# Xiuyu-Li/q-diffusion

Hardware: NVIDIA H100
Metric: images_per_sec (higher is better)
Workload: dtype int8 (W4/W8 codes x A8 codes, int32 accumulate; fp32 norms/softmax)

## Files before the change

q-diffusion_b200/csrc/attention_wg.cuh:

```cuda
#pragma once
#include "attention.cuh"
#include "ptx.cuh"

namespace qd {

__device__ __forceinline__ void wgmma_ra_s8s8_n64(uint32_t* d, const uint32_t (&a)[4], uint64_t db, uint32_t scale_d) {
  asm volatile(
      "{\n\t.reg .pred p;\n\t"
      "setp.ne.b32 p, %37, 0;\n\t"
      "wgmma.mma_async.sync.aligned.m64n64k32.s32.s8.s8 "
      "{%0, %1, %2, %3, %4, %5, %6, %7, %8, %9, %10, %11, %12, %13, %14, %15, %16, %17, %18, %19, %20, %21, %22, %23, %24, %25, %26, %27, %28, %29, %30, %31}, {%32, %33, %34, %35}, %36, p;\n\t}\n"
      : "+r"(d[0]), "+r"(d[1]), "+r"(d[2]), "+r"(d[3]), "+r"(d[4]), "+r"(d[5]), "+r"(d[6]), "+r"(d[7]), "+r"(d[8]), "+r"(d[9]), "+r"(d[10]), "+r"(d[11]), "+r"(d[12]), "+r"(d[13]), "+r"(d[14]), "+r"(d[15]), "+r"(d[16]), "+r"(d[17]), "+r"(d[18]), "+r"(d[19]), "+r"(d[20]), "+r"(d[21]), "+r"(d[22]), "+r"(d[23]), "+r"(d[24]), "+r"(d[25]), "+r"(d[26]), "+r"(d[27]), "+r"(d[28]), "+r"(d[29]), "+r"(d[30]), "+r"(d[31])
      : "r"(a[0]), "r"(a[1]), "r"(a[2]), "r"(a[3]), "l"(db), "r"(scale_d));
}
__device__ __forceinline__ void wgmma_ra_u8u8_n64(uint32_t* d, const uint32_t (&a)[4], uint64_t db, uint32_t scale_d) {
  asm volatile(
      "{\n\t.reg .pred p;\n\t"
      "setp.ne.b32 p, %37, 0;\n\t"
      "wgmma.mma_async.sync.aligned.m64n64k32.s32.u8.u8 "
      "{%0, %1, %2, %3, %4, %5, %6, %7, %8, %9, %10, %11, %12, %13, %14, %15, %16, %17, %18, %19, %20, %21, %22, %23, %24, %25, %26, %27, %28, %29, %30, %31}, {%32, %33, %34, %35}, %36, p;\n\t}\n"
      : "+r"(d[0]), "+r"(d[1]), "+r"(d[2]), "+r"(d[3]), "+r"(d[4]), "+r"(d[5]), "+r"(d[6]), "+r"(d[7]), "+r"(d[8]), "+r"(d[9]), "+r"(d[10]), "+r"(d[11]), "+r"(d[12]), "+r"(d[13]), "+r"(d[14]), "+r"(d[15]), "+r"(d[16]), "+r"(d[17]), "+r"(d[18]), "+r"(d[19]), "+r"(d[20]), "+r"(d[21]), "+r"(d[22]), "+r"(d[23]), "+r"(d[24]), "+r"(d[25]), "+r"(d[26]), "+r"(d[27]), "+r"(d[28]), "+r"(d[29]), "+r"(d[30]), "+r"(d[31])
      : "r"(a[0]), "r"(a[1]), "r"(a[2]), "r"(a[3]), "l"(db), "r"(scale_d));
}
__device__ __forceinline__ void wgmma_ra_f16_n64(float* d, const uint32_t (&a)[4], uint64_t db, uint32_t scale_d) {
  asm volatile(
      "{\n\t.reg .pred p;\n\t"
      "setp.ne.b32 p, %37, 0;\n\t"
      "wgmma.mma_async.sync.aligned.m64n64k16.f32.f16.f16 "
      "{%0, %1, %2, %3, %4, %5, %6, %7, %8, %9, %10, %11, %12, %13, %14, %15, %16, %17, %18, %19, %20, %21, %22, %23, %24, %25, %26, %27, %28, %29, %30, %31}, {%32, %33, %34, %35}, %36, p, 1, 1, 0;\n\t}\n"
      : "+f"(d[0]), "+f"(d[1]), "+f"(d[2]), "+f"(d[3]), "+f"(d[4]), "+f"(d[5]), "+f"(d[6]), "+f"(d[7]), "+f"(d[8]), "+f"(d[9]), "+f"(d[10]), "+f"(d[11]), "+f"(d[12]), "+f"(d[13]), "+f"(d[14]), "+f"(d[15]), "+f"(d[16]), "+f"(d[17]), "+f"(d[18]), "+f"(d[19]), "+f"(d[20]), "+f"(d[21]), "+f"(d[22]), "+f"(d[23]), "+f"(d[24]), "+f"(d[25]), "+f"(d[26]), "+f"(d[27]), "+f"(d[28]), "+f"(d[29]), "+f"(d[30]), "+f"(d[31])
      : "r"(a[0]), "r"(a[1]), "r"(a[2]), "r"(a[3]), "l"(db), "r"(scale_d));
}
__device__ __forceinline__ void wgmma_ra_u8u8_n24(uint32_t* d, const uint32_t (&a)[4], uint64_t db, uint32_t scale_d) {
  asm volatile(
      "{\n\t.reg .pred p;\n\t"
      "setp.ne.b32 p, %17, 0;\n\t"
      "wgmma.mma_async.sync.aligned.m64n24k32.s32.u8.u8 "
      "{%0, %1, %2, %3, %4, %5, %6, %7, %8, %9, %10, %11}, {%12, %13, %14, %15}, %16, p;\n\t}\n"
      : "+r"(d[0]), "+r"(d[1]), "+r"(d[2]), "+r"(d[3]), "+r"(d[4]), "+r"(d[5]), "+r"(d[6]), "+r"(d[7]), "+r"(d[8]), "+r"(d[9]), "+r"(d[10]), "+r"(d[11])
      : "r"(a[0]), "r"(a[1]), "r"(a[2]), "r"(a[3]), "l"(db), "r"(scale_d));
}
__device__ __forceinline__ void wgmma_ra_u8s8_n24(uint32_t* d, const uint32_t (&a)[4], uint64_t db, uint32_t scale_d) {
  asm volatile(
      "{\n\t.reg .pred p;\n\t"
      "setp.ne.b32 p, %17, 0;\n\t"
      "wgmma.mma_async.sync.aligned.m64n24k32.s32.u8.s8 "
      "{%0, %1, %2, %3, %4, %5, %6, %7, %8, %9, %10, %11}, {%12, %13, %14, %15}, %16, p;\n\t}\n"
      : "+r"(d[0]), "+r"(d[1]), "+r"(d[2]), "+r"(d[3]), "+r"(d[4]), "+r"(d[5]), "+r"(d[6]), "+r"(d[7]), "+r"(d[8]), "+r"(d[9]), "+r"(d[10]), "+r"(d[11])
      : "r"(a[0]), "r"(a[1]), "r"(a[2]), "r"(a[3]), "l"(db), "r"(scale_d));
}
__device__ __forceinline__ void wgmma_ra_u8u8_n32(uint32_t* d, const uint32_t (&a)[4], uint64_t db, uint32_t scale_d) {
  asm volatile(
      "{\n\t.reg .pred p;\n\t"
      "setp.ne.b32 p, %21, 0;\n\t"
      "wgmma.mma_async.sync.aligned.m64n32k32.s32.u8.u8 "
      "{%0, %1, %2, %3, %4, %5, %6, %7, %8, %9, %10, %11, %12, %13, %14, %15}, {%16, %17, %18, %19}, %20, p;\n\t}\n"
      : "+r"(d[0]), "+r"(d[1]), "+r"(d[2]), "+r"(d[3]), "+r"(d[4]), "+r"(d[5]), "+r"(d[6]), "+r"(d[7]), "+r"(d[8]), "+r"(d[9]), "+r"(d[10]), "+r"(d[11]), "+r"(d[12]), "+r"(d[13]), "+r"(d[14]), "+r"(d[15])
      : "r"(a[0]), "r"(a[1]), "r"(a[2]), "r"(a[3]), "l"(db), "r"(scale_d));
}
__device__ __forceinline__ void wgmma_ra_u8s8_n32(uint32_t* d, const uint32_t (&a)[4], uint64_t db, uint32_t scale_d) {
  asm volatile(
      "{\n\t.reg .pred p;\n\t"
      "setp.ne.b32 p, %21, 0;\n\t"
      "wgmma.mma_async.sync.aligned.m64n32k32.s32.u8.s8 "
      "{%0, %1, %2, %3, %4, %5, %6, %7, %8, %9, %10, %11, %12, %13, %14, %15}, {%16, %17, %18, %19}, %20, p;\n\t}\n"
      : "+r"(d[0]), "+r"(d[1]), "+r"(d[2]), "+r"(d[3]), "+r"(d[4]), "+r"(d[5]), "+r"(d[6]), "+r"(d[7]), "+r"(d[8]), "+r"(d[9]), "+r"(d[10]), "+r"(d[11]), "+r"(d[12]), "+r"(d[13]), "+r"(d[14]), "+r"(d[15])
      : "r"(a[0]), "r"(a[1]), "r"(a[2]), "r"(a[3]), "l"(db), "r"(scale_d));
}
__device__ __forceinline__ void wgmma_ra_u8u8_n48(uint32_t* d, const uint32_t (&a)[4], uint64_t db, uint32_t scale_d) {
  asm volatile(
      "{\n\t.reg .pred p;\n\t"
      "setp.ne.b32 p, %29, 0;\n\t"
      "wgmma.mma_async.sync.aligned.m64n48k32.s32.u8.u8 "
      "{%0, %1, %2, %3, %4, %5, %6, %7, %8, %9, %10, %11, %12, %13, %14, %15, %16, %17, %18, %19, %20, %21, %22, %23}, {%24, %25, %26, %27}, %28, p;\n\t}\n"
      : "+r"(d[0]), "+r"(d[1]), "+r"(d[2]), "+r"(d[3]), "+r"(d[4]), "+r"(d[5]), "+r"(d[6]), "+r"(d[7]), "+r"(d[8]), "+r"(d[9]), "+r"(d[10]), "+r"(d[11]), "+r"(d[12]), "+r"(d[13]), "+r"(d[14]), "+r"(d[15]), "+r"(d[16]), "+r"(d[17]), "+r"(d[18]), "+r"(d[19]), "+r"(d[20]), "+r"(d[21]), "+r"(d[22]), "+r"(d[23])
      : "r"(a[0]), "r"(a[1]), "r"(a[2]), "r"(a[3]), "l"(db), "r"(scale_d));
}
__device__ __forceinline__ void wgmma_ra_u8s8_n48(uint32_t* d, const uint32_t (&a)[4], uint64_t db, uint32_t scale_d) {
  asm volatile(
      "{\n\t.reg .pred p;\n\t"
      "setp.ne.b32 p, %29, 0;\n\t"
      "wgmma.mma_async.sync.aligned.m64n48k32.s32.u8.s8 "
      "{%0, %1, %2, %3, %4, %5, %6, %7, %8, %9, %10, %11, %12, %13, %14, %15, %16, %17, %18, %19, %20, %21, %22, %23}, {%24, %25, %26, %27}, %28, p;\n\t}\n"
      : "+r"(d[0]), "+r"(d[1]), "+r"(d[2]), "+r"(d[3]), "+r"(d[4]), "+r"(d[5]), "+r"(d[6]), "+r"(d[7]), "+r"(d[8]), "+r"(d[9]), "+r"(d[10]), "+r"(d[11]), "+r"(d[12]), "+r"(d[13]), "+r"(d[14]), "+r"(d[15]), "+r"(d[16]), "+r"(d[17]), "+r"(d[18]), "+r"(d[19]), "+r"(d[20]), "+r"(d[21]), "+r"(d[22]), "+r"(d[23])
      : "r"(a[0]), "r"(a[1]), "r"(a[2]), "r"(a[3]), "l"(db), "r"(scale_d));
}
__device__ __forceinline__ void wgmma_ra_u8s8_n64(uint32_t* d, const uint32_t (&a)[4], uint64_t db, uint32_t scale_d) {
  asm volatile(
      "{\n\t.reg .pred p;\n\t"
      "setp.ne.b32 p, %37, 0;\n\t"
      "wgmma.mma_async.sync.aligned.m64n64k32.s32.u8.s8 "
      "{%0, %1, %2, %3, %4, %5, %6, %7, %8, %9, %10, %11, %12, %13, %14, %15, %16, %17, %18, %19, %20, %21, %22, %23, %24, %25, %26, %27, %28, %29, %30, %31}, {%32, %33, %34, %35}, %36, p;\n\t}\n"
      : "+r"(d[0]), "+r"(d[1]), "+r"(d[2]), "+r"(d[3]), "+r"(d[4]), "+r"(d[5]), "+r"(d[6]), "+r"(d[7]), "+r"(d[8]), "+r"(d[9]), "+r"(d[10]), "+r"(d[11]), "+r"(d[12]), "+r"(d[13]), "+r"(d[14]), "+r"(d[15]), "+r"(d[16]), "+r"(d[17]), "+r"(d[18]), "+r"(d[19]), "+r"(d[20]), "+r"(d[21]), "+r"(d[22]), "+r"(d[23]), "+r"(d[24]), "+r"(d[25]), "+r"(d[26]), "+r"(d[27]), "+r"(d[28]), "+r"(d[29]), "+r"(d[30]), "+r"(d[31])
      : "r"(a[0]), "r"(a[1]), "r"(a[2]), "r"(a[3]), "l"(db), "r"(scale_d));
}
__device__ __forceinline__ void wgmma_ra_u8u8_n80(uint32_t* d, const uint32_t (&a)[4], uint64_t db, uint32_t scale_d) {
  asm volatile(
      "{\n\t.reg .pred p;\n\t"
      "setp.ne.b32 p, %45, 0;\n\t"
      "wgmma.mma_async.sync.aligned.m64n80k32.s32.u8.u8 "
      "{%0, %1, %2, %3, %4, %5, %6, %7, %8, %9, %10, %11, %12, %13, %14, %15, %16, %17, %18, %19, %20, %21, %22, %23, %24, %25, %26, %27, %28, %29, %30, %31, %32, %33, %34, %35, %36, %37, %38, %39}, {%40, %41, %42, %43}, %44, p;\n\t}\n"
      : "+r"(d[0]), "+r"(d[1]), "+r"(d[2]), "+r"(d[3]), "+r"(d[4]), "+r"(d[5]), "+r"(d[6]), "+r"(d[7]), "+r"(d[8]), "+r"(d[9]), "+r"(d[10]), "+r"(d[11]), "+r"(d[12]), "+r"(d[13]), "+r"(d[14]), "+r"(d[15]), "+r"(d[16]), "+r"(d[17]), "+r"(d[18]), "+r"(d[19]), "+r"(d[20]), "+r"(d[21]), "+r"(d[22]), "+r"(d[23]), "+r"(d[24]), "+r"(d[25]), "+r"(d[26]), "+r"(d[27]), "+r"(d[28]), "+r"(d[29]), "+r"(d[30]), "+r"(d[31]), "+r"(d[32]), "+r"(d[33]), "+r"(d[34]), "+r"(d[35]), "+r"(d[36]), "+r"(d[37]), "+r"(d[38]), "+r"(d[39])
      : "r"(a[0]), "r"(a[1]), "r"(a[2]), "r"(a[3]), "l"(db), "r"(scale_d));
}
__device__ __forceinline__ void wgmma_ra_u8s8_n80(uint32_t* d, const uint32_t (&a)[4], uint64_t db, uint32_t scale_d) {
  asm volatile(
      "{\n\t.reg .pred p;\n\t"
      "setp.ne.b32 p, %45, 0;\n\t"
      "wgmma.mma_async.sync.aligned.m64n80k32.s32.u8.s8 "
      "{%0, %1, %2, %3, %4, %5, %6, %7, %8, %9, %10, %11, %12, %13, %14, %15, %16, %17, %18, %19, %20, %21, %22, %23, %24, %25, %26, %27, %28, %29, %30, %31, %32, %33, %34, %35, %36, %37, %38, %39}, {%40, %41, %42, %43}, %44, p;\n\t}\n"
      : "+r"(d[0]), "+r"(d[1]), "+r"(d[2]), "+r"(d[3]), "+r"(d[4]), "+r"(d[5]), "+r"(d[6]), "+r"(d[7]), "+r"(d[8]), "+r"(d[9]), "+r"(d[10]), "+r"(d[11]), "+r"(d[12]), "+r"(d[13]), "+r"(d[14]), "+r"(d[15]), "+r"(d[16]), "+r"(d[17]), "+r"(d[18]), "+r"(d[19]), "+r"(d[20]), "+r"(d[21]), "+r"(d[22]), "+r"(d[23]), "+r"(d[24]), "+r"(d[25]), "+r"(d[26]), "+r"(d[27]), "+r"(d[28]), "+r"(d[29]), "+r"(d[30]), "+r"(d[31]), "+r"(d[32]), "+r"(d[33]), "+r"(d[34]), "+r"(d[35]), "+r"(d[36]), "+r"(d[37]), "+r"(d[38]), "+r"(d[39])
      : "r"(a[0]), "r"(a[1]), "r"(a[2]), "r"(a[3]), "l"(db), "r"(scale_d));
}
__device__ __forceinline__ void wgmma_ra_u8u8_n96(uint32_t* d, const uint32_t (&a)[4], uint64_t db, uint32_t scale_d) {
  asm volatile(
      "{\n\t.reg .pred p;\n\t"
      "setp.ne.b32 p, %53, 0;\n\t"
      "wgmma.mma_async.sync.aligned.m64n96k32.s32.u8.u8 "
      "{%0, %1, %2, %3, %4, %5, %6, %7, %8, %9, %10, %11, %12, %13, %14, %15, %16, %17, %18, %19, %20, %21, %22, %23, %24, %25, %26, %27, %28, %29, %30, %31, %32, %33, %34, %35, %36, %37, %38, %39, %40, %41, %42, %43, %44, %45, %46, %47}, {%48, %49, %50, %51}, %52, p;\n\t}\n"
      : "+r"(d[0]), "+r"(d[1]), "+r"(d[2]), "+r"(d[3]), "+r"(d[4]), "+r"(d[5]), "+r"(d[6]), "+r"(d[7]), "+r"(d[8]), "+r"(d[9]), "+r"(d[10]), "+r"(d[11]), "+r"(d[12]), "+r"(d[13]), "+r"(d[14]), "+r"(d[15]), "+r"(d[16]), "+r"(d[17]), "+r"(d[18]), "+r"(d[19]), "+r"(d[20]), "+r"(d[21]), "+r"(d[22]), "+r"(d[23]), "+r"(d[24]), "+r"(d[25]), "+r"(d[26]), "+r"(d[27]), "+r"(d[28]), "+r"(d[29]), "+r"(d[30]), "+r"(d[31]), "+r"(d[32]), "+r"(d[33]), "+r"(d[34]), "+r"(d[35]), "+r"(d[36]), "+r"(d[37]), "+r"(d[38]), "+r"(d[39]), "+r"(d[40]), "+r"(d[41]), "+r"(d[42]), "+r"(d[43]), "+r"(d[44]), "+r"(d[45]), "+r"(d[46]), "+r"(d[47])
      : "r"(a[0]), "r"(a[1]), "r"(a[2]), "r"(a[3]), "l"(db), "r"(scale_d));
}
__device__ __forceinline__ void wgmma_ra_u8s8_n96(uint32_t* d, const uint32_t (&a)[4], uint64_t db, uint32_t scale_d) {
  asm volatile(
      "{\n\t.reg .pred p;\n\t"
      "setp.ne.b32 p, %53, 0;\n\t"
      "wgmma.mma_async.sync.aligned.m64n96k32.s32.u8.s8 "
      "{%0, %1, %2, %3, %4, %5, %6, %7, %8, %9, %10, %11, %12, %13, %14, %15, %16, %17, %18, %19, %20, %21, %22, %23, %24, %25, %26, %27, %28, %29, %30, %31, %32, %33, %34, %35, %36, %37, %38, %39, %40, %41, %42, %43, %44, %45, %46, %47}, {%48, %49, %50, %51}, %52, p;\n\t}\n"
      : "+r"(d[0]), "+r"(d[1]), "+r"(d[2]), "+r"(d[3]), "+r"(d[4]), "+r"(d[5]), "+r"(d[6]), "+r"(d[7]), "+r"(d[8]), "+r"(d[9]), "+r"(d[10]), "+r"(d[11]), "+r"(d[12]), "+r"(d[13]), "+r"(d[14]), "+r"(d[15]), "+r"(d[16]), "+r"(d[17]), "+r"(d[18]), "+r"(d[19]), "+r"(d[20]), "+r"(d[21]), "+r"(d[22]), "+r"(d[23]), "+r"(d[24]), "+r"(d[25]), "+r"(d[26]), "+r"(d[27]), "+r"(d[28]), "+r"(d[29]), "+r"(d[30]), "+r"(d[31]), "+r"(d[32]), "+r"(d[33]), "+r"(d[34]), "+r"(d[35]), "+r"(d[36]), "+r"(d[37]), "+r"(d[38]), "+r"(d[39]), "+r"(d[40]), "+r"(d[41]), "+r"(d[42]), "+r"(d[43]), "+r"(d[44]), "+r"(d[45]), "+r"(d[46]), "+r"(d[47])
      : "r"(a[0]), "r"(a[1]), "r"(a[2]), "r"(a[3]), "l"(db), "r"(scale_d));
}
__device__ __forceinline__ void wgmma_ra_u8u8_n112(uint32_t* d, const uint32_t (&a)[4], uint64_t db, uint32_t scale_d) {
  asm volatile(
      "{\n\t.reg .pred p;\n\t"
      "setp.ne.b32 p, %61, 0;\n\t"
      "wgmma.mma_async.sync.aligned.m64n112k32.s32.u8.u8 "
      "{%0, %1, %2, %3, %4, %5, %6, %7, %8, %9, %10, %11, %12, %13, %14, %15, %16, %17, %18, %19, %20, %21, %22, %23, %24, %25, %26, %27, %28, %29, %30, %31, %32, %33, %34, %35, %36, %37, %38, %39, %40, %41, %42, %43, %44, %45, %46, %47, %48, %49, %50, %51, %52, %53, %54, %55}, {%56, %57, %58, %59}, %60, p;\n\t}\n"
      : "+r"(d[0]), "+r"(d[1]), "+r"(d[2]), "+r"(d[3]), "+r"(d[4]), "+r"(d[5]), "+r"(d[6]), "+r"(d[7]), "+r"(d[8]), "+r"(d[9]), "+r"(d[10]), "+r"(d[11]), "+r"(d[12]), "+r"(d[13]), "+r"(d[14]), "+r"(d[15]), "+r"(d[16]), "+r"(d[17]), "+r"(d[18]), "+r"(d[19]), "+r"(d[20]), "+r"(d[21]), "+r"(d[22]), "+r"(d[23]), "+r"(d[24]), "+r"(d[25]), "+r"(d[26]), "+r"(d[27]), "+r"(d[28]), "+r"(d[29]), "+r"(d[30]), "+r"(d[31]), "+r"(d[32]), "+r"(d[33]), "+r"(d[34]), "+r"(d[35]), "+r"(d[36]), "+r"(d[37]), "+r"(d[38]), "+r"(d[39]), "+r"(d[40]), "+r"(d[41]), "+r"(d[42]), "+r"(d[43]), "+r"(d[44]), "+r"(d[45]), "+r"(d[46]), "+r"(d[47]), "+r"(d[48]), "+r"(d[49]), "+r"(d[50]), "+r"(d[51]), "+r"(d[52]), "+r"(d[53]), "+r"(d[54]), "+r"(d[55])
      : "r"(a[0]), "r"(a[1]), "r"(a[2]), "r"(a[3]), "l"(db), "r"(scale_d));
}
__device__ __forceinline__ void wgmma_ra_u8s8_n112(uint32_t* d, const uint32_t (&a)[4], uint64_t db, uint32_t scale_d) {
  asm volatile(
      "{\n\t.reg .pred p;\n\t"
      "setp.ne.b32 p, %61, 0;\n\t"
      "wgmma.mma_async.sync.aligned.m64n112k32.s32.u8.s8 "
      "{%0, %1, %2, %3, %4, %5, %6, %7, %8, %9, %10, %11, %12, %13, %14, %15, %16, %17, %18, %19, %20, %21, %22, %23, %24, %25, %26, %27, %28, %29, %30, %31, %32, %33, %34, %35, %36, %37, %38, %39, %40, %41, %42, %43, %44, %45, %46, %47, %48, %49, %50, %51, %52, %53, %54, %55}, {%56, %57, %58, %59}, %60, p;\n\t}\n"
      : "+r"(d[0]), "+r"(d[1]), "+r"(d[2]), "+r"(d[3]), "+r"(d[4]), "+r"(d[5]), "+r"(d[6]), "+r"(d[7]), "+r"(d[8]), "+r"(d[9]), "+r"(d[10]), "+r"(d[11]), "+r"(d[12]), "+r"(d[13]), "+r"(d[14]), "+r"(d[15]), "+r"(d[16]), "+r"(d[17]), "+r"(d[18]), "+r"(d[19]), "+r"(d[20]), "+r"(d[21]), "+r"(d[22]), "+r"(d[23]), "+r"(d[24]), "+r"(d[25]), "+r"(d[26]), "+r"(d[27]), "+r"(d[28]), "+r"(d[29]), "+r"(d[30]), "+r"(d[31]), "+r"(d[32]), "+r"(d[33]), "+r"(d[34]), "+r"(d[35]), "+r"(d[36]), "+r"(d[37]), "+r"(d[38]), "+r"(d[39]), "+r"(d[40]), "+r"(d[41]), "+r"(d[42]), "+r"(d[43]), "+r"(d[44]), "+r"(d[45]), "+r"(d[46]), "+r"(d[47]), "+r"(d[48]), "+r"(d[49]), "+r"(d[50]), "+r"(d[51]), "+r"(d[52]), "+r"(d[53]), "+r"(d[54]), "+r"(d[55])
      : "r"(a[0]), "r"(a[1]), "r"(a[2]), "r"(a[3]), "l"(db), "r"(scale_d));
}

constexpr int ATW_STAGES = 4;
constexpr int ATW_THREADS = ATT_WARPS * 32;
__host__ __device__ constexpr int atw_nv(int DV) {
  return DV + 8 <= 24 ? 24 : DV + 8 <= 32 ? 32 : DV + 8 <= 48 ? 48 : DV + 8 <= 64 ? 64 : DV + 8 <= 80 ? 80 : DV + 8 <= 96 ? 96 : 112;
}
struct AtwSmem {
  int k_bytes, v_bytes, z_off, bar_off, total;
};
__host__ __device__ inline AtwSmem atw_smem(int P, int NV) {
  AtwSmem l;
  l.k_bytes = (ATT_BN * P + 1023) / 1024 * 1024;
  l.v_bytes = (NV * ATT_BN + 1023) / 1024 * 1024;
  l.z_off = ATW_STAGES * (l.k_bytes + l.v_bytes);
  l.bar_off = l.z_off + ATW_STAGES * ATT_BN * 4;
  l.total = l.bar_off + ATW_STAGES * 8 + ATW_STAGES * 4 + 1024;
  return l;
}
__device__ __forceinline__ uint64_t atw_desc(uint32_t addr, int row_bytes) {
  const uint64_t layout = row_bytes == 128 ? 1 : row_bytes == 64 ? 2 : 3;
  uint64_t d = (uint64_t)((addr & 0x3FFFF) >> 4);
  d |= (uint64_t)1 << 16;
  d |= (uint64_t)((8 * row_bytes) >> 4) << 32;
  d |= layout << 62;
  return d;
}

template <int N, bool VS>
__device__ __forceinline__ void atw_pv(uint32_t* d, const uint32_t (&a)[4], uint64_t db, uint32_t scale_d) {
  if constexpr (VS) {
    if constexpr (N == 24) wgmma_ra_u8s8_n24(d, a, db, scale_d);
    else if constexpr (N == 32) wgmma_ra_u8s8_n32(d, a, db, scale_d);
    else if constexpr (N == 48) wgmma_ra_u8s8_n48(d, a, db, scale_d);
    else if constexpr (N == 64) wgmma_ra_u8s8_n64(d, a, db, scale_d);
    else if constexpr (N == 80) wgmma_ra_u8s8_n80(d, a, db, scale_d);
    else if constexpr (N == 96) wgmma_ra_u8s8_n96(d, a, db, scale_d);
    else wgmma_ra_u8s8_n112(d, a, db, scale_d);
  } else {
    if constexpr (N == 24) wgmma_ra_u8u8_n24(d, a, db, scale_d);
    else if constexpr (N == 32) wgmma_ra_u8u8_n32(d, a, db, scale_d);
    else if constexpr (N == 48) wgmma_ra_u8u8_n48(d, a, db, scale_d);
    else if constexpr (N == 64) wgmma_ra_u8u8_n64(d, a, db, scale_d);
    else if constexpr (N == 80) wgmma_ra_u8u8_n80(d, a, db, scale_d);
    else if constexpr (N == 96) wgmma_ra_u8u8_n96(d, a, db, scale_d);
    else wgmma_ra_u8u8_n112(d, a, db, scale_d);
  }
}

template <int DQ, int DV, bool QK_SIGNED, bool V_SIGNED, bool SM16, bool F16, int MINB>
__global__ void __launch_bounds__(ATW_THREADS, MINB)
qattention_wg_kernel(const __grid_constant__ CUtensorMap tmK, const __grid_constant__ CUtensorMap tmV,
                     const qd_attention_desc p, int P) {
  constexpr int NV = atw_nv(DV);
  constexpr int NKC = DQ / 32;
  constexpr int NDT = DV / 8 + 1;
  constexpr int RB = F16 ? 2 * DV : DV;
  static_assert(!F16 || DV <= 64, "fp16 Q / K operands: d <= 64 keeps |S| below 2^22");
  static_assert(DV <= 96, "8-bit codes: the raw scores must stay below 2^23 (unsigned) / 2^22 (signed)");
  using SV = std::conditional_t<F16, float, uint32_t>;
  constexpr uint32_t MB = QK_SIGNED ? 0x4B400000u : 0x4B000000u;
  extern __shared__ uint8_t atw_raw[];
  uint8_t* smem = atw_raw + (((smem_u32(atw_raw) + 1023u) & ~1023u) - smem_u32(atw_raw));
  const AtwSmem lay = atw_smem(P, NV);
  uint64_t* full = reinterpret_cast<uint64_t*>(smem + lay.bar_off);
  int* released = reinterpret_cast<int*>(full + ATW_STAGES);

  const int warp = threadIdx.x >> 5, lane = threadIdx.x & 31;
  const int g = lane >> 2, t = lane & 3;
  const int bh = blockIdx.y;
  const int b = bh / p.heads, h = bh - b * p.heads;
  const int row0 = blockIdx.x * ATT_BM + warp * 16;
  const int ntiles = (p.Tk + ATT_BN - 1) / ATT_BN;
  const int nloads = 2 * ntiles;
  const bool has_zq = !F16 && p.zq != 0;
  const int* zrk_g = reinterpret_cast<const int*>(p.ws) + (long long)bh * (long long)att_ws_stride(p.Tk);

  for (int i = threadIdx.x; i < ATW_STAGES * (NV - DV) * ATT_BN; i += ATW_THREADS) {
    const int s = i / ((NV - DV) * ATT_BN), r = (i / ATT_BN) % (NV - DV) + DV, c = i % ATT_BN;
    smem[ATW_STAGES * lay.k_bytes + s * lay.v_bytes + r * ATT_BN + c] = r == DV ? 1 : 0;
  }
  if (threadIdx.x == 0) {
    tma_prefetch_desc(&tmK);
    tma_prefetch_desc(&tmV);
    for (int s = 0; s < ATW_STAGES; ++s) {
      mbar_init(&full[s], 1);
      released[s] = 0;
    }
    fence_mbar_init();
  }
  fence_proxy_async();
  __syncthreads();

  auto issue = [&](int L) {
    const int s = L % ATW_STAGES, pass = L / ntiles, tile = L - pass * ntiles;
    const int j0 = tile * ATT_BN;
    const uint32_t bytes = (uint32_t)(ATT_BN * P) + (pass ? (uint32_t)(ATT_BN * DV) : 0u) + (has_zq ? ATT_BN * 4u : 0u);
    mbar_arrive_expect_tx(&full[s], bytes);
    tma_load_2d(smem + s * lay.k_bytes, &tmK, &full[s], h * P, b * p.Tk + j0);
    if (pass) tma_load_2d(smem + ATW_STAGES * lay.k_bytes + s * lay.v_bytes, &tmV, &full[s], j0, bh * DV);
    if (has_zq) bulk_load_1d(smem + lay.z_off + s * ATT_BN * 4, zrk_g + j0, ATT_BN * 4, &full[s]);
  };
  if (threadIdx.x == 0)
    for (int L = 0; L < ATW_STAGES && L < nloads; ++L) issue(L);

  constexpr bool QRELOAD = DV == 48;
  uint32_t qf[NKC][4];
  const uint8_t* qbase = reinterpret_cast<const uint8_t*>(p.q) + (long long)b * p.Tq * p.ld_q + p.q_off + h * p.head_stride_q;
  const uint8_t* q0 = qbase + (long long)min(row0 + g, p.Tq - 1) * p.ld_q;
  const uint8_t* q1 = qbase + (long long)min(row0 + g + 8, p.Tq - 1) * p.ld_q;
  auto load_q = [&]() {
#pragma unroll
    for (int kc = 0; kc < NKC; ++kc) {
      const int c0 = kc * 32 + 4 * t, c1 = c0 + 16;
      qf[kc][0] = c0 < RB ? *reinterpret_cast<const uint32_t*>(q0 + c0) : 0u;
      qf[kc][1] = c0 < RB ? *reinterpret_cast<const uint32_t*>(q1 + c0) : 0u;
      qf[kc][2] = c1 < RB ? *reinterpret_cast<const uint32_t*>(q0 + c1) : 0u;
      qf[kc][3] = c1 < RB ? *reinterpret_cast<const uint32_t*>(q1 + c1) : 0u;
    }
  };
  if constexpr (!QRELOAD) load_q();
  const float c = p.sim_scale * 1.4426950408889634f;
  const bool ragged = (p.Tk % ATT_BN) != 0;
  float mi0 = -INFINITY, mi1 = -INFINITY;
  float l0 = 0.f, l1 = 0.f;

  auto issue_s = [&](SV (&s)[8][4], int L) {
    const int st = L % ATW_STAGES;
    if constexpr (QRELOAD) load_q();
    mbar_wait(&full[st], (uint32_t)(L / ATW_STAGES) & 1u);
    const uint64_t dK = atw_desc(smem_u32(smem + st * lay.k_bytes), P);
    wgmma_fence();
#pragma unroll
    for (int kc = 0; kc < NKC; ++kc) {
      if constexpr (F16) wgmma_ra_f16_n64(&s[0][0], qf[kc], dK + (uint64_t)(2 * kc), kc ? 1u : 0u);
      else if constexpr (QK_SIGNED) wgmma_ra_s8s8_n64(&s[0][0], qf[kc], dK + (uint64_t)(2 * kc), kc ? 1u : 0u);
      else wgmma_ra_u8u8_n64(&s[0][0], qf[kc], dK + (uint64_t)(2 * kc), kc ? 1u : 0u);
    }
    wgmma_commit();
  };
  auto scores = [&](SV (&s)[8][4], float (&f)[8][4], int L) {
    wgmma_fence_regs(reinterpret_cast<SV (&)[32]>(s));
    const int tile = L % ntiles, st = L % ATW_STAGES;
    if constexpr (F16) {
#pragma unroll
      for (int i = 0; i < 32; ++i) f[i >> 2][i & 3] = s[i >> 2][i & 3];
    } else {
      const uint32_t* sZrk = reinterpret_cast<const uint32_t*>(smem + lay.z_off + st * ATT_BN * 4);
#pragma unroll
      for (int nt = 0; nt < 8; ++nt) {
        float z0 = __uint_as_float(MB), z1 = z0;
        if (has_zq) {
          const uint2 z = *reinterpret_cast<const uint2*>(sZrk + 8 * nt + 2 * t);
          z0 = __uint_as_float(z.x + MB);
          z1 = __uint_as_float(z.y + MB);
        }
        f[nt][0] = __uint_as_float(s[nt][0] + MB) - z0; f[nt][1] = __uint_as_float(s[nt][1] + MB) - z1;
        f[nt][2] = __uint_as_float(s[nt][2] + MB) - z0; f[nt][3] = __uint_as_float(s[nt][3] + MB) - z1;
      }
    }
    if (ragged && tile == ntiles - 1) {
#pragma unroll
      for (int nt = 0; nt < 8; ++nt) {
        const int j = tile * ATT_BN + 8 * nt + 2 * t;
        if (j >= p.Tk) { f[nt][0] = -INFINITY; f[nt][2] = -INFINITY; }
        if (j + 1 >= p.Tk) { f[nt][1] = -INFINITY; f[nt][3] = -INFINITY; }
      }
    }
  };

  auto release = [&](int R) {
    __syncwarp();
    if (lane == 0) {
      const int s = R % ATW_STAGES;
      __threadfence_block();
      const int n = atomicAdd(&released[s], 1);
      if (n == ATT_WARPS * (R / ATW_STAGES + 1) - 1 && R + ATW_STAGES < nloads) {
        __threadfence_block();
        issue(R + ATW_STAGES);
      }
    }
  };

  for (int L = 0; L < ntiles; ++L) {
    SV sacc[8][4];
    issue_s(sacc, L);
    wgmma_wait<0>();
    float f[8][4];
    scores(sacc, f, L);
    release(L);
    float tm0 = f[0][0], tm1 = f[0][2];
#pragma unroll
    for (int nt = 0; nt < 8; ++nt) {
      tm0 = fmaxf(tm0, fmaxf(f[nt][0], f[nt][1]));
      tm1 = fmaxf(tm1, fmaxf(f[nt][2], f[nt][3]));
    }
    tm0 = fmaxf(tm0, __shfl_xor_sync(0xffffffffu, tm0, 1));
    tm0 = fmaxf(tm0, __shfl_xor_sync(0xffffffffu, tm0, 2));
    tm1 = fmaxf(tm1, __shfl_xor_sync(0xffffffffu, tm1, 1));
    tm1 = fmaxf(tm1, __shfl_xor_sync(0xffffffffu, tm1, 2));
    if (tm0 > mi0) { l0 *= (mi0 == -INFINITY) ? 0.f : ex2_approx((mi0 - tm0) * c); mi0 = tm0; }
    if (tm1 > mi1) { l1 *= (mi1 == -INFINITY) ? 0.f : ex2_approx((mi1 - tm1) * c); mi1 = tm1; }
    const float b0 = -mi0 * c, b1 = -mi1 * c;
    float a0 = 0.f, a1 = 0.f;
#pragma unroll
    for (int nt = 0; nt < 8; ++nt) {
      a0 += ex2_approx(fmaf(f[nt][0], c, b0)) + ex2_approx(fmaf(f[nt][1], c, b0));
      a1 += ex2_approx(fmaf(f[nt][2], c, b1)) + ex2_approx(fmaf(f[nt][3], c, b1));
    }
    l0 += a0;
    l1 += a1;
  }

  l0 += __shfl_xor_sync(0xffffffffu, l0, 1);
  l0 += __shfl_xor_sync(0xffffffffu, l0, 2);
  l1 += __shfl_xor_sync(0xffffffffu, l1, 1);
  l1 += __shfl_xor_sync(0xffffffffu, l1, 2);
  const float off0 = -mi0 * c + log2f(1.0f / (l0 * p.delta_w));
  const float off1 = -mi1 * c + log2f(1.0f / (l1 * p.delta_w));
  const float pmax = (float)p.p_qmax;
// ... 84 lines not shown
```

q-diffusion_b200/csrc/engine.cu:

```cuda
#include <cuda.h>
#include <cuda_runtime.h>
#include <cudaTypedefs.h>

#include <atomic>
#include <cstdarg>
#include <cstdio>
#include <cstdlib>
#include <cstring>
#include <mutex>
#include <new>
#include <utility>
#include <vector>

#include "../../include/qdiff_b200.h"
#include "attention.cuh"
#include "attention_wg.cuh"
#include "elem.cuh"
#include "gemm_i8.cuh"
#include "runtime.cuh"

namespace qdr {

thread_local char g_err[512] = "";
std::atomic<long long> g_launches{0};
// ... 664 lines not shown
bool im2col_vec(const qd_im2col_desc& d) {
  return (d.C % 16) == 0 && d.ld_dst == 9 * d.C && (d.ld_dst % 16) == 0 && aligned(d.src, 16) && aligned(d.dst, 16);
}

int validate_im2col(const qd_im2col_desc& d) {
  if (!d.src || !d.dst) return fail(QD_ERR_BAD_ARG, "im2col: null arg");
  if (d.B <= 0 || d.H <= 0 || d.W <= 0 || d.C <= 0 || d.Ho <= 0 || d.Wo <= 0 || d.stride <= 0)
    return fail(QD_ERR_BAD_ARG, "im2col: empty geometry");
  if (d.ld_dst < 9 * d.C) return fail(QD_ERR_BAD_ARG, "im2col: ld_dst too small");
  return QD_OK;
}

int launch_im2col(const qd_im2col_desc& d, cudaStream_t s) {
  if (int rc = validate_im2col(d)) return rc;
  if (im2col_vec(d)) {
    launch_k(qd::im2col_vec_kernel, grid_for((long long)d.B * d.Ho * d.Wo * 9 * (d.C / 16), 256), 256, 0, s, d);
    return check_launch("im2col_vec_kernel");
  }
  const long long total = (long long)d.B * d.Ho * d.Wo * d.ld_dst;
  launch_k(qd::im2col_kernel, grid_for(total, 256), 256, 0, s, d);
  return check_launch("im2col_kernel");
}

template <int DQ, int DV, bool QS, bool VS, bool S16, bool F16>
int launch_attention_inst(const qd_attention_desc& d, cudaStream_t s) {
  constexpr int MINB = (DV <= 48) ? 2 : 1;
  auto kern = qd::qattention_kernel<DQ, DV, QS, VS, S16, MINB, F16>;
  static std::atomic<unsigned long long> optin{0};
  if (int rc = ensure_smem_optin(kern, 200 * 1024, optin, "attention")) return rc;
  const bool zrk = !F16 && d.zq != 0;
  const qd::AttSmemLayout lay = qd::att_smem_layout(DQ, DV, d.Tk, zrk);
  if (lay.total > 200 * 1024) return fail(QD_ERR_UNSUPPORTED, "attention: Tk=%d needs %d B of shared memory", d.Tk, lay.total);
  if (zrk) {
    if (!d.ws) return fail(QD_ERR_BAD_ARG, "attention: workspace required when zq != 0");
    const int tk_pad = qd::att_ws_stride(d.Tk);
    launch_k(qd::att_krowsum_kernel<QS>, grid_for((long long)d.B * d.heads * tk_pad, 256), 256, 0, s, d, tk_pad, 0, 0);
    int rc = check_launch("att_krowsum_kernel");
    if (rc) return rc;
  }
  dim3 grid((d.Tq + qd::ATT_BM - 1) / qd::ATT_BM, d.B * d.heads);
  launch_k(kern, grid, qd::ATT_WARPS * 32, lay.total, s, d);
  return check_launch("qattention_kernel");
}

template <int DQ, int DV, bool F16 = false>
int launch_attention_t(const qd_attention_desc& d, cudaStream_t s) {
  const bool qs = d.q_signed != 0, vs = d.v_signed != 0, s16 = d.sm_bits > 8;
  if (qs && vs && s16) return launch_attention_inst<DQ, DV, true, true, true, F16>(d, s);
  if (qs && vs && !s16) return launch_attention_inst<DQ, DV, true, true, false, F16>(d, s);
  if (!qs && !vs && s16) return launch_attention_inst<DQ, DV, false, false, true, F16>(d, s);
  if (!qs && !vs && !s16) return launch_attention_inst<DQ, DV, false, false, false, F16>(d, s);
  return fail(QD_ERR_UNSUPPORTED, "attention: mixed signedness q=%d v=%d", d.q_signed, d.v_signed);
}

template <int DQ, int DV, bool QS, bool VS, bool S16>
int launch_attention_smallk_inst(const qd_attention_desc& d, cudaStream_t s) {
  constexpr int NKV = 3;
  auto kern = qd::qattention_smallk_kernel<DQ, DV, QS, VS, S16, NKV>;
  const int spw = d.Tq >= 2048 ? 4 : (d.Tq >= 512 ? 2 : 1);
  const int slabs = (d.Tq + 15) / 16;
  dim3 grid((slabs + spw * qd::ATS_WARPS - 1) / (spw * qd::ATS_WARPS), d.B * d.heads);
  launch_k(kern, grid, qd::ATS_WARPS * 32, qd::ats_smem_bytes<DQ, DV, NKV>(), s, d, spw);
  return check_launch("qattention_smallk_kernel");
}

template <int DQ, int DV>
int launch_attention_smallk(const qd_attention_desc& d, cudaStream_t s) {
  const bool qs = d.q_signed != 0, vs = d.v_signed != 0, s16 = d.sm_bits > 8;
  if (qs && vs && s16) return launch_attention_smallk_inst<DQ, DV, true, true, true>(d, s);
  if (qs && vs && !s16) return launch_attention_smallk_inst<DQ, DV, true, true, false>(d, s);
  if (!qs && !vs && s16) return launch_attention_smallk_inst<DQ, DV, false, false, true>(d, s);
  if (!qs && !vs && !s16) return launch_attention_smallk_inst<DQ, DV, false, false, false>(d, s);
  return fail(QD_ERR_UNSUPPORTED, "attention: mixed signedness q=%d v=%d", d.q_signed, d.v_signed);
}

bool attention_wg_eligible(const qd_attention_desc& d) {
  static const int forced_mma = [] { const char* e = getenv("QDIFF_ATTENTION"); return (e && !strcmp(e, "mma")) ? 1 : 0; }();
  if (forced_mma) return false;
  const int P = d.head_stride_q, rb = d.qk_f16 ? 2 * d.d : d.d;
  if (d.d != 16 && d.d != 24 && d.d != 32 && d.d != 40 && d.d != 48 && d.d != 64 && d.d != 80 && d.d != 96) return false;
  if (d.qk_f16 && d.d > 64) return false;
  if ((P != 32 && P != 64 && P != 128) || P < rb || d.head_stride_k != P) return false;
  if (d.q_off != 0 || d.k_off != 0 || (d.ld_k & 15) || (((uintptr_t)d.k) & 15) || (((uintptr_t)d.vt) & 15)) return false;
  if (d.v_off != 0 || d.head_stride_v != d.d || d.v_batch_stride != (long long)d.heads * d.d * d.ld_vt) return false;
  if (d.zq != 0 && !d.qk_f16 && !d.ws) return false;
  if (!d.qk_f16 && (d.zq > 255 || d.zq < (d.q_signed ? -255 : 0))) return false;
  return true;
}

template <int DQ, int DV, bool QS, bool VS, bool S16, bool F16>
int launch_attention_wg_inst(const qd_attention_desc& d, cudaStream_t s) {
  constexpr int MINB = DV <= 40 ? 2 : 1;
  auto kern = qd::qattention_wg_kernel<DQ, DV, QS, VS, S16, F16, MINB>;
  const int P = d.head_stride_q;
  const qd::AtwSmem lay = qd::atw_smem(P, qd::atw_nv(DV));
  static std::atomic<unsigned long long> optin{0};
  if (int rc = ensure_smem_optin(kern, 227 * 1024, optin, "attention_wg")) return rc;
  CUtensorMap tmK, tmV;
  {
    cuuint64_t dims[2] = {(cuuint64_t)d.ld_k, (cuuint64_t)d.B * d.Tk};
    cuuint64_t strides[1] = {(cuuint64_t)d.ld_k};
    cuuint32_t box[2] = {(cuuint32_t)P, (cuuint32_t)qd::ATT_BN};
    if (int rc = encode_u8_map(&tmK, d.k, 2, dims, strides, box, P)) return rc;
  }
  {
    cuuint64_t dims[2] = {(cuuint64_t)d.ld_vt, (cuuint64_t)d.B * d.heads * d.d};
    cuuint64_t strides[1] = {(cuuint64_t)d.ld_vt};
    cuuint32_t box[2] = {(cuuint32_t)qd::ATT_BN, (cuuint32_t)d.d};
    if (int rc = encode_u8_map(&tmV, d.vt, 2, dims, strides, box, 64)) return rc;
  }
  if (!F16 && d.zq != 0) {
    const int tk_pad = qd::att_ws_stride(d.Tk);
    launch_k(qd::att_krowsum_kernel<QS>, grid_for((long long)d.B * d.heads * tk_pad, 256), 256, 0, s, d, tk_pad, 0, 0);
    if (int rc = check_launch("att_krowsum_kernel")) return rc;
  }
  dim3 grid((d.Tq + qd::ATT_BM - 1) / qd::ATT_BM, d.B * d.heads);
  launch_k(kern, grid, qd::ATW_THREADS, lay.total, s, tmK, tmV, d, P);
  return check_launch("qattention_wg_kernel");
}

template <int DQ, int DV, bool F16>
int launch_attention_wg_t(const qd_attention_desc& d, cudaStream_t s) {
  const bool qs = d.q_signed != 0, vs = d.v_signed != 0, s16 = d.sm_bits > 8;
  if (qs && vs && s16) return launch_attention_wg_inst<DQ, DV, true, true, true, F16>(d, s);
  if (qs && vs && !s16) return launch_attention_wg_inst<DQ, DV, true, true, false, F16>(d, s);
  if (!qs && !vs && s16) return launch_attention_wg_inst<DQ, DV, false, false, true, F16>(d, s);
  if (!qs && !vs && !s16) return launch_attention_wg_inst<DQ, DV, false, false, false, F16>(d, s);
  return fail(QD_ERR_UNSUPPORTED, "attention: mixed signedness q=%d v=%d", d.q_signed, d.v_signed);
}

int launch_attention_wg(const qd_attention_desc& d, cudaStream_t s) {
  if (d.qk_f16) {
    switch (d.d) {
      case 16: return launch_attention_wg_t<32, 16, true>(d, s);
      case 24: return launch_attention_wg_t<64, 24, true>(d, s);
      case 32: return launch_attention_wg_t<64, 32, true>(d, s);
      case 40: return launch_attention_wg_t<96, 40, true>(d, s);
      case 48: return launch_attention_wg_t<96, 48, true>(d, s);
      default: return launch_attention_wg_t<128, 64, true>(d, s);
    }
  }
  switch (d.d) {
    case 16: return launch_attention_wg_t<32, 16, false>(d, s);
    case 24: return launch_attention_wg_t<32, 24, false>(d, s);
    case 32: return launch_attention_wg_t<32, 32, false>(d, s);
    case 40: return launch_attention_wg_t<64, 40, false>(d, s);
    case 48: return launch_attention_wg_t<64, 48, false>(d, s);
    case 64: return launch_attention_wg_t<64, 64, false>(d, s);
    case 80: return launch_attention_wg_t<96, 80, false>(d, s);
    default: return launch_attention_wg_t<96, 96, false>(d, s);
  }
}

int validate_attention(const qd_attention_desc& d) {
  if (!d.q || !d.k || !d.vt || (!d.out && !d.out_q)) return fail(QD_ERR_BAD_ARG, "attention: null arg");
  if (d.out_q && (d.ld_out_q & 1)) return fail(QD_ERR_UNSUPPORTED, "attention: ld_out_q");
  if (d.q_signed != d.k_signed) return fail(QD_ERR_UNSUPPORTED, "attention: q/k signedness differ");
  if (d.zw != 0) return fail(QD_ERR_UNSUPPORTED, "attention: softmax zero point must be 0 (got %d)", d.zw);
  if (d.sm_bits != 8 && d.sm_bits != 16) return fail(QD_ERR_UNSUPPORTED, "attention: sm_bits %d", d.sm_bits);
  if (!(d.sim_scale > 0.f)) return fail(QD_ERR_UNSUPPORTED, "attention: sim_scale must be positive (got %g)", d.sim_scale);
  if (!d.qk_f16 && d.d > 64 &&
      (2147483648.0 - 65025.0 * d.d) * d.sim_scale * 1.4426950408889634 < 128.0 + fmax(0.0, -log2((double)d.delta_w)))
    return fail(QD_ERR_UNSUPPORTED, "attention: sim_scale %g too small to mask the keys beyond Tk at d = %d", d.sim_scale, d.d);
  if (d.ld_vt % 16 || d.ld_vt < d.Tk) return fail(QD_ERR_BAD_ARG, "attention: ld_vt");
  if ((d.q_off | d.head_stride_q | (int)d.ld_q) & 3) return fail(QD_ERR_UNSUPPORTED, "attention: q needs 4-byte alignment");
  if ((d.k_off | d.head_stride_k | (int)d.ld_k | d.d) & 7) return fail(QD_ERR_UNSUPPORTED, "attention: k rows need 8-byte alignment");
  if (d.out && (d.ld_out % 2)) return fail(QD_ERR_UNSUPPORTED, "attention: ld_out");
  return QD_OK;
}

int launch_attention(const qd_attention_desc& d, cudaStream_t s) {
  if (int rc = validate_attention(d)) return rc;
  if (d.qk_f16) {
    if (attention_wg_eligible(d)) return launch_attention_wg(d, s);
    switch (d.d) {
      case 16: return launch_attention_t<32, 16, true>(d, s);
      case 24: return launch_attention_t<64, 24, true>(d, s);
      case 32: return launch_attention_t<64, 32, true>(d, s);
      case 40: return launch_attention_t<96, 40, true>(d, s);
      case 48: return launch_attention_t<96, 48, true>(d, s);
      case 64: return launch_attention_t<128, 64, true>(d, s);
      default: return fail(QD_ERR_UNSUPPORTED, "attention: qk_f16 needs d in {16, 24, 32, 40, 48, 64} (got %d)", d.d);
    }
  }
  if (d.Tk <= 96 && (d.d == 40 || d.d == 80)) {
    static const bool off = [] { const char* e = getenv("QDIFF_ATTENTION"); return e && !strcmp(e, "nosmallk"); }();
    if (!off) return d.d == 40 ? launch_attention_smallk<64, 40>(d, s) : launch_attention_smallk<96, 80>(d, s);
  }
  if (attention_wg_eligible(d)) return launch_attention_wg(d, s);
  switch (d.d) {
    case 16: return launch_attention_t<32, 16>(d, s);
    case 24: return launch_attention_t<32, 24>(d, s);
    case 32: return launch_attention_t<32, 32>(d, s);
    case 40: return launch_attention_t<64, 40>(d, s);
    case 48: return launch_attention_t<64, 48>(d, s);
    case 64: return launch_attention_t<64, 64>(d, s);
    case 80: return launch_attention_t<96, 80>(d, s);
    case 96: return launch_attention_t<96, 96>(d, s);
    case 160: return launch_attention_t<160, 160>(d, s);
    case 256: return launch_attention_t<256, 256>(d, s);
// ... 284 lines not shown
```

Before: 4.545.

## Stage Q tile in shared memory via TMA for DV=48 attention and use SS wgmma

For head dim 48, the attention kernel previously reloaded Q fragments from global memory into registers on every K tile to save registers. It now loads the Q block once into swizzled shared memory with a TMA load on its own mbarrier, zero-pads the columns beyond the real head dim, and issues shared-memory-operand wgmma for QK^T. This removes the repeated global Q loads and the register pressure of holding Q, at the cost of extra shared memory per block and a new alignment eligibility check on Q.

Measured after the change: 4.551, median of 6. Within noise of the previous version (+0.1%).

```diff
diff --git a/q-diffusion_b200/csrc/attention_wg.cuh b/q-diffusion_b200/csrc/attention_wg.cuh
--- a/q-diffusion_b200/csrc/attention_wg.cuh
+++ b/q-diffusion_b200/csrc/attention_wg.cuh
@@ -3,6 +3,25 @@
 #include "ptx.cuh"
 
 namespace qd {
+
+__device__ __forceinline__ void wgmma_ss_u8u8_n64(uint32_t* d, uint64_t da, uint64_t db, uint32_t scale_d) {
+  asm volatile(
+      "{\n\t.reg .pred p;\n\t"
+      "setp.ne.b32 p, %34, 0;\n\t"
+      "wgmma.mma_async.sync.aligned.m64n64k32.s32.u8.u8 "
+      "{%0, %1, %2, %3, %4, %5, %6, %7, %8, %9, %10, %11, %12, %13, %14, %15, %16, %17, %18, %19, %20, %21, %22, %23, %24, %25, %26, %27, %28, %29, %30, %31}, %32, %33, p;\n\t}\n"
+      : "+r"(d[0]), "+r"(d[1]), "+r"(d[2]), "+r"(d[3]), "+r"(d[4]), "+r"(d[5]), "+r"(d[6]), "+r"(d[7]), "+r"(d[8]), "+r"(d[9]), "+r"(d[10]), "+r"(d[11]), "+r"(d[12]), "+r"(d[13]), "+r"(d[14]), "+r"(d[15]), "+r"(d[16]), "+r"(d[17]), "+r"(d[18]), "+r"(d[19]), "+r"(d[20]), "+r"(d[21]), "+r"(d[22]), "+r"(d[23]), "+r"(d[24]), "+r"(d[25]), "+r"(d[26]), "+r"(d[27]), "+r"(d[28]), "+r"(d[29]), "+r"(d[30]), "+r"(d[31])
+      : "l"(da), "l"(db), "r"(scale_d));
+}
+__device__ __forceinline__ void wgmma_ss_f16_n64(float* d, uint64_t da, uint64_t db, uint32_t scale_d) {
+  asm volatile(
+      "{\n\t.reg .pred p;\n\t"
+      "setp.ne.b32 p, %34, 0;\n\t"
+      "wgmma.mma_async.sync.aligned.m64n64k16.f32.f16.f16 "
+      "{%0, %1, %2, %3, %4, %5, %6, %7, %8, %9, %10, %11, %12, %13, %14, %15, %16, %17, %18, %19, %20, %21, %22, %23, %24, %25, %26, %27, %28, %29, %30, %31}, %32, %33, p, 1, 1, 0, 0;\n\t}\n"
+      : "+f"(d[0]), "+f"(d[1]), "+f"(d[2]), "+f"(d[3]), "+f"(d[4]), "+f"(d[5]), "+f"(d[6]), "+f"(d[7]), "+f"(d[8]), "+f"(d[9]), "+f"(d[10]), "+f"(d[11]), "+f"(d[12]), "+f"(d[13]), "+f"(d[14]), "+f"(d[15]), "+f"(d[16]), "+f"(d[17]), "+f"(d[18]), "+f"(d[19]), "+f"(d[20]), "+f"(d[21]), "+f"(d[22]), "+f"(d[23]), "+f"(d[24]), "+f"(d[25]), "+f"(d[26]), "+f"(d[27]), "+f"(d[28]), "+f"(d[29]), "+f"(d[30]), "+f"(d[31])
+      : "l"(da), "l"(db), "r"(scale_d));
+}
 
 __device__ __forceinline__ void wgmma_ra_s8s8_n64(uint32_t* d, const uint32_t (&a)[4], uint64_t db, uint32_t scale_d) {
   asm volatile(
@@ -154,16 +173,18 @@
 __host__ __device__ constexpr int atw_nv(int DV) {
   return DV + 8 <= 24 ? 24 : DV + 8 <= 32 ? 32 : DV + 8 <= 48 ? 48 : DV + 8 <= 64 ? 64 : DV + 8 <= 80 ? 80 : DV + 8 <= 96 ? 96 : 112;
 }
+__host__ __device__ constexpr bool atw_q_smem(int DV) { return DV == 48; }
 struct AtwSmem {
-  int k_bytes, v_bytes, z_off, bar_off, total;
+  int k_bytes, v_bytes, q_off, z_off, bar_off, total;
 };
-__host__ __device__ inline AtwSmem atw_smem(int P, int NV) {
+__host__ __device__ inline AtwSmem atw_smem(int P, int NV, bool q_smem) {
   AtwSmem l;
   l.k_bytes = (ATT_BN * P + 1023) / 1024 * 1024;
   l.v_bytes = (NV * ATT_BN + 1023) / 1024 * 1024;
-  l.z_off = ATW_STAGES * (l.k_bytes + l.v_bytes);
+  l.q_off = ATW_STAGES * (l.k_bytes + l.v_bytes);
+  l.z_off = l.q_off + (q_smem ? (ATT_BM * P + 1023) / 1024 * 1024 : 0);
   l.bar_off = l.z_off + ATW_STAGES * ATT_BN * 4;
-  l.total = l.bar_off + ATW_STAGES * 8 + ATW_STAGES * 4 + 1024;
+  l.total = l.bar_off + (ATW_STAGES + 1) * 8 + ATW_STAGES * 4 + 1024;
   return l;
 }
 __device__ __forceinline__ uint64_t atw_desc(uint32_t addr, int row_bytes) {
@@ -198,8 +219,8 @@
 
 template <int DQ, int DV, bool QK_SIGNED, bool V_SIGNED, bool SM16, bool F16, int MINB>
 __global__ void __launch_bounds__(ATW_THREADS, MINB)
-qattention_wg_kernel(const __grid_constant__ CUtensorMap tmK, const __grid_constant__ CUtensorMap tmV,
-                     const qd_attention_desc p, int P) {
+qattention_wg_kernel(const __grid_constant__ CUtensorMap tmQ, const __grid_constant__ CUtensorMap tmK,
+                     const __grid_constant__ CUtensorMap tmV, const qd_attention_desc p, int P) {
   constexpr int NV = atw_nv(DV);
   constexpr int NKC = DQ / 32;
   constexpr int NDT = DV / 8 + 1;
@@ -210,9 +231,11 @@
   constexpr uint32_t MB = QK_SIGNED ? 0x4B400000u : 0x4B000000u;
   extern __shared__ uint8_t atw_raw[];
   uint8_t* smem = atw_raw + (((smem_u32(atw_raw) + 1023u) & ~1023u) - smem_u32(atw_raw));
-  const AtwSmem lay = atw_smem(P, NV);
+  constexpr bool QS = atw_q_smem(DV);
+  const AtwSmem lay = atw_smem(P, NV, QS);
   uint64_t* full = reinterpret_cast<uint64_t*>(smem + lay.bar_off);
-  int* released = reinterpret_cast<int*>(full + ATW_STAGES);
+  uint64_t* qbar = full + ATW_STAGES;
+  int* released = reinterpret_cast<int*>(full + ATW_STAGES + 1);
 
   const int warp = threadIdx.x >> 5, lane = threadIdx.x & 31;
   const int g = lane >> 2, t = lane & 3;
@@ -229,12 +252,14 @@
     smem[ATW_STAGES * lay.k_bytes + s * lay.v_bytes + r * ATT_BN + c] = r == DV ? 1 : 0;
   }
   if (threadIdx.x == 0) {
+    if constexpr (QS) tma_prefetch_desc(&tmQ);
     tma_prefetch_desc(&tmK);
     tma_prefetch_desc(&tmV);
     for (int s = 0; s < ATW_STAGES; ++s) {
       mbar_init(&full[s], 1);
       released[s] = 0;
     }
+    mbar_init(qbar, 1);
     fence_mbar_init();
   }
   fence_proxy_async();
@@ -249,15 +274,33 @@
     if (pass) tma_load_2d(smem + ATW_STAGES * lay.k_bytes + s * lay.v_bytes, &tmV, &full[s], j0, bh * DV);
     if (has_zq) bulk_load_1d(smem + lay.z_off + s * ATT_BN * 4, zrk_g + j0, ATT_BN * 4, &full[s]);
   };
-  if (threadIdx.x == 0)
+  if (threadIdx.x == 0) {
+    if constexpr (QS) {
+      mbar_arrive_expect_tx(qbar, (uint32_t)(ATT_BM * P));
+      tma_load_2d(smem + lay.q_off, &tmQ, qbar, h * P, b * p.Tq + blockIdx.x * ATT_BM);
+    }
     for (int L = 0; L < ATW_STAGES && L < nloads; ++L) issue(L);
-
-  constexpr bool QRELOAD = DV == 48;
-  uint32_t qf[NKC][4];
-  const uint8_t* qbase = reinterpret_cast<const uint8_t*>(p.q) + (long long)b * p.Tq * p.ld_q + p.q_off + h * p.head_stride_q;
-  const uint8_t* q0 = qbase + (long long)min(row0 + g, p.Tq - 1) * p.ld_q;
-  const uint8_t* q1 = qbase + (long long)min(row0 + g + 8, p.Tq - 1) * p.ld_q;
-  auto load_q = [&]() {
+  }
+
+  uint32_t qf[QS ? 1 : NKC][4];
+  uint64_t dQ = 0;
+  if constexpr (QS) {
+    mbar_wait(qbar, 0);
+    if constexpr (RB < DQ) {
+      constexpr int NZ = (DQ - RB) / 8;
+      const int sw = P / 16 - 1;
+      for (int i = threadIdx.x; i < ATT_BM * NZ; i += ATW_THREADS) {
+        const int o = (i / NZ) * P + RB + 8 * (i % NZ);
+        *reinterpret_cast<uint2*>(smem + lay.q_off + (o ^ (((o >> 7) & sw) << 4))) = make_uint2(0u, 0u);
+      }
+      fence_proxy_async();
+    }
+    __syncthreads();
+    dQ = atw_desc(smem_u32(smem + lay.q_off + (warp >> 2) * 64 * P), P);
+  } else {
+    const uint8_t* qbase = reinterpret_cast<const uint8_t*>(p.q) + (long long)b * p.Tq * p.ld_q + p.q_off + h * p.head_stride_q;
+    const uint8_t* q0 = qbase + (long long)min(row0 + g, p.Tq - 1) * p.ld_q;
+    const uint8_t* q1 = qbase + (long long)min(row0 + g + 8, p.Tq - 1) * p.ld_q;
 #pragma unroll
     for (int kc = 0; kc < NKC; ++kc) {
       const int c0 = kc * 32 + 4 * t, c1 = c0 + 16;
@@ -266,8 +309,7 @@
       qf[kc][2] = c1 < RB ? *reinterpret_cast<const uint32_t*>(q0 + c1) : 0u;
       qf[kc][3] = c1 < RB ? *reinterpret_cast<const uint32_t*>(q1 + c1) : 0u;
     }
-  };
-  if constexpr (!QRELOAD) load_q();
+  }
   const float c = p.sim_scale * 1.4426950408889634f;
   const bool ragged = (p.Tk % ATT_BN) != 0;
   float mi0 = -INFINITY, mi1 = -INFINITY;
@@ -275,15 +317,22 @@
 
   auto issue_s = [&](SV (&s)[8][4], int L) {
     const int st = L % ATW_STAGES;
-    if constexpr (QRELOAD) load_q();
     mbar_wait(&full[st], (uint32_t)(L / ATW_STAGES) & 1u);
     const uint64_t dK = atw_desc(smem_u32(smem + st * lay.k_bytes), P);
     wgmma_fence();
 #pragma unroll
     for (int kc = 0; kc < NKC; ++kc) {
-      if constexpr (F16) wgmma_ra_f16_n64(&s[0][0], qf[kc], dK + (uint64_t)(2 * kc), kc ? 1u : 0u);
-      else if constexpr (QK_SIGNED) wgmma_ra_s8s8_n64(&s[0][0], qf[kc], dK + (uint64_t)(2 * kc), kc ? 1u : 0u);
-      else wgmma_ra_u8u8_n64(&s[0][0], qf[kc], dK + (uint64_t)(2 * kc), kc ? 1u : 0u);
+      const uint64_t dKk = dK + (uint64_t)(2 * kc);
+      if constexpr (QS) {
+        const uint64_t dQk = dQ + (uint64_t)(2 * kc);
+        if constexpr (F16) wgmma_ss_f16_n64(&s[0][0], dQk, dKk, kc ? 1u : 0u);
+        else if constexpr (QK_SIGNED) wgmma_s8s8_n64(reinterpret_cast<uint32_t (&)[32]>(s), dQk, dKk, kc ? 1u : 0u);
+        else wgmma_ss_u8u8_n64(&s[0][0], dQk, dKk, kc ? 1u : 0u);
+      } else {
+        if constexpr (F16) wgmma_ra_f16_n64(&s[0][0], qf[kc], dKk, kc ? 1u : 0u);
+        else if constexpr (QK_SIGNED) wgmma_ra_s8s8_n64(&s[0][0], qf[kc], dKk, kc ? 1u : 0u);
+        else wgmma_ra_u8u8_n64(&s[0][0], qf[kc], dKk, kc ? 1u : 0u);
+      }
     }
     wgmma_commit();
   };
diff --git a/q-diffusion_b200/csrc/engine.cu b/q-diffusion_b200/csrc/engine.cu
--- a/q-diffusion_b200/csrc/engine.cu
+++ b/q-diffusion_b200/csrc/engine.cu
@@ -770,6 +770,7 @@
   if (d.qk_f16 && d.d > 64) return false;
   if ((P != 32 && P != 64 && P != 128) || P < rb || d.head_stride_k != P) return false;
   if (d.q_off != 0 || d.k_off != 0 || (d.ld_k & 15) || (((uintptr_t)d.k) & 15) || (((uintptr_t)d.vt) & 15)) return false;
+  if (d.d == 48 && ((d.ld_q & 15) || (((uintptr_t)d.q) & 15))) return false;
   if (d.v_off != 0 || d.head_stride_v != d.d || d.v_batch_stride != (long long)d.heads * d.d * d.ld_vt) return false;
   if (d.zq != 0 && !d.qk_f16 && !d.ws) return false;
   if (!d.qk_f16 && (d.zq > 255 || d.zq < (d.q_signed ? -255 : 0))) return false;
@@ -781,10 +782,11 @@
   constexpr int MINB = DV <= 40 ? 2 : 1;
   auto kern = qd::qattention_wg_kernel<DQ, DV, QS, VS, S16, F16, MINB>;
   const int P = d.head_stride_q;
-  const qd::AtwSmem lay = qd::atw_smem(P, qd::atw_nv(DV));
+  constexpr bool QSMEM = qd::atw_q_smem(DV);
+  const qd::AtwSmem lay = qd::atw_smem(P, qd::atw_nv(DV), QSMEM);
   static std::atomic<unsigned long long> optin{0};
   if (int rc = ensure_smem_optin(kern, 227 * 1024, optin, "attention_wg")) return rc;
-  CUtensorMap tmK, tmV;
+  CUtensorMap tmQ, tmK, tmV;
   {
     cuuint64_t dims[2] = {(cuuint64_t)d.ld_k, (cuuint64_t)d.B * d.Tk};
     cuuint64_t strides[1] = {(cuuint64_t)d.ld_k};
@@ -797,13 +799,21 @@
     cuuint32_t box[2] = {(cuuint32_t)qd::ATT_BN, (cuuint32_t)d.d};
     if (int rc = encode_u8_map(&tmV, d.vt, 2, dims, strides, box, 64)) return rc;
   }
+  if (QSMEM) {
+    cuuint64_t dims[2] = {(cuuint64_t)d.ld_q, (cuuint64_t)d.B * d.Tq};
+    cuuint64_t strides[1] = {(cuuint64_t)d.ld_q};
+    cuuint32_t box[2] = {(cuuint32_t)P, (cuuint32_t)qd::ATT_BM};
+    if (int rc = encode_u8_map(&tmQ, d.q, 2, dims, strides, box, P)) return rc;
+  } else {
+    tmQ = tmK;
+  }
   if (!F16 && d.zq != 0) {
     const int tk_pad = qd::att_ws_stride(d.Tk);
     launch_k(qd::att_krowsum_kernel<QS>, grid_for((long long)d.B * d.heads * tk_pad, 256), 256, 0, s, d, tk_pad, 0, 0);
     if (int rc = check_launch("att_krowsum_kernel")) return rc;
   }
   dim3 grid((d.Tq + qd::ATT_BM - 1) / qd::ATT_BM, d.B * d.heads);
-  launch_k(kern, grid, qd::ATW_THREADS, lay.total, s, tmK, tmV, d, P);
+  launch_k(kern, grid, qd::ATW_THREADS, lay.total, s, tmQ, tmK, tmV, d, P);
   return check_launch("qattention_wg_kernel");
 }
 
```
